# jgrss/cultionet

Hardware: AMD Instinct MI355X
Metric: train_chips_per_sec (higher is better)
Workload: dtype f32

## Files before the change

### cultionet_amd/csrc/cn_wgrad.hip

```cpp
#include <cstdlib>
#include "cn_common.h"
#include "cn_profile.h"
#include "cn_slicesum.h"

#define WG_MAX_TAPS 9
#define WG_BC 32
#define WG_NS 4
#define WG_NB 13
#define WG_KS 8
#define WG_U 4
#define WG_KB 16

struct CnWgradGeom {
  int N;
  int A, Hs, Ws; long sbs; long scs;
  int Bc, Hb, Wb; long bbs; long bcs;
  double flops;
  int s;
  int T;
  int offy[WG_MAX_TAPS], offx[WG_MAX_TAPS];
  int min_oy, min_ox;
  long sa;
  int PR, Wsp, pitch_s;
  int rows_b, pitch_b, plane_b;
  int a_tiles;
  int chunks_per_img, total_chunks, chunks_per_split;
  int b_lds_off;
  int buf_stride;
  int nbuf;
  int colsplit;
  int G, spg;
  const float* gS[4];
  const float* gB[4];
  float* gdW[4];
  long slice_stride;
  int grid_x, grid_y, grid_z;
  int mq_lo, mq_hi;
};

typedef __attribute__((address_space(3))) void* cn_lds_ptr;
typedef const __attribute__((address_space(1))) void* cn_gbl_ptr;

__device__ float cn_zero_line[64];

__device__ __forceinline__ void cn_glds4(const float* src, float* lds_wave_base) {
  __builtin_amdgcn_global_load_lds((cn_gbl_ptr)src, (cn_lds_ptr)lds_wave_base, 4, 0, 0);
}

template <int T>
__global__ __launch_bounds__(256) void cn_wgrad_kernel(const float* __restrict__ S, const float* __restrict__ Bg,
                                                      float* __restrict__ dW, const CnWgradGeom g) {
  extern __shared__ __attribute__((aligned(16))) float smem[];

  const int tid = threadIdx.x, lane = tid & 63, wid = tid >> 6;
  const int half = lane >> 5, l31 = lane & 31;
  const int at = wid % g.a_tiles, kp = wid / g.a_tiles, kparts = 4 / g.a_tiles;
  int bx, by, bz;
  if (!cn_xcd_block(g.grid_x, g.grid_y, g.grid_x * g.grid_y * g.grid_z, bx, by, bz)) return;
  const int a0 = by * g.a_tiles * 32;
  const int b0 = bx * WG_BC;
  const int npix = g.PR * g.Wsp;
  const float* zero = cn_zero_line + lane;

  int so[WG_NS];
#pragma unroll
  for (int i = 0; i < WG_NS; ++i) {
    const int e = lane + i * 64;
    if (e < npix) {
      const int r = e / g.Wsp, c = e - r * g.Wsp;
      so[i] = (r << 16) | ((c < g.Ws) ? c : 0xFFFF);
    } else {
      so[i] = -2;
    }
  }
  int bo[WG_NB];
#pragma unroll
  for (int i = 0; i < WG_NB; ++i) {
    const int e = lane + i * 64;
    if (e < g.plane_b) {
      const int r = e / g.pitch_b;
      bo[i] = (r << 16) | (e - r * g.pitch_b);
    } else {
      bo[i] = -1;
    }
  }

  int boff[T];
#pragma unroll
  for (int j = 0; j < T; ++j) {
    const int n = j * 32 + l31;
    const int bl = n / T, t = n - bl * T;
    boff[j] = bl * g.plane_b + (g.offy[t] - g.min_oy) * g.pitch_b + (g.offx[t] - g.min_ox) + half * g.s;
  }
  const int aoff = (at * 32 + l31) * g.pitch_s + half;

  f32x16 acc[T];
#pragma unroll
  for (int j = 0; j < T; ++j)
#pragma unroll
    for (int r = 0; r < 16; ++r) acc[j][r] = 0.f;

  const int HWs = g.Hs * g.Ws, HWb = g.Hb * g.Wb;
  const int arows = g.a_tiles * 32;
  int chunk = bz * g.chunks_per_split;
  int chunk_end = chunk + g.chunks_per_split;
  if (chunk_end > g.total_chunks) chunk_end = g.total_chunks;

  const int steps = npix >> 1;
  const int q_begin = (steps * kp) / kparts, q_end = (steps * (kp + 1)) / kparts;
  const int e_begin = q_begin * 2;
  const int r_begin = e_begin / g.Wsp, c_begin = e_begin - r_begin * g.Wsp;

  auto stage = [&](int ck, int buf) {
    float* s_lds = smem + buf * g.buf_stride;
    float* b_lds = s_lds + g.b_lds_off;
    const int n = ck / g.chunks_per_img;
    const int gy0 = (ck - n * g.chunks_per_img) * g.PR;
    const int pr = (g.Hs - gy0 < g.PR) ? g.Hs - gy0 : g.PR;
    const float* Sn = S + (long)n * g.sbs + (long)gy0 * g.Ws;
    for (int a = wid; a < arows; a += 4) {
      const bool aok = (a0 + a) < g.A;
      const float* Sa = Sn + (long)(a0 + a) * g.scs;
#pragma unroll
      for (int i = 0; i < WG_NS; ++i) {
        if (i * 64 < npix) {
          if (so[i] != -2) {
            const int r = so[i] >> 16, c = so[i] & 0xFFFF;
            const float* src = (aok && c != 0xFFFF && r < pr) ? Sa + r * g.Ws + c : zero;
            cn_glds4(src, s_lds + a * g.pitch_s + i * 64);
          }
        }
      }
    }
    const float* Bn = Bg + (long)n * g.bbs;
    const int iy0 = gy0 * g.s + g.min_oy;
    for (int bl = wid; bl < WG_BC; bl += 4) {
      const bool bok = (b0 + bl) < g.Bc;
      const float* Bb = Bn + (long)(b0 + bl) * g.bcs;
#pragma unroll
      for (int i = 0; i < WG_NB; ++i) {
        if (i * 64 < g.plane_b) {
          if (bo[i] >= 0) {
            const int iy = iy0 + (bo[i] >> 16), ix = g.min_ox + (bo[i] & 0xFFFF);
            const float* src = (bok && iy >= 0 && iy < g.Hb && ix >= 0 && ix < g.Wb) ? Bb + iy * g.Wb + ix : zero;
            cn_glds4(src, b_lds + bl * g.plane_b + i * 64);
          }
        }
      }
    }
  };

  int cur = 0;
  if (chunk < chunk_end && g.nbuf == 2) stage(chunk, 0);
  for (; chunk < chunk_end; ++chunk) {
    if (g.nbuf == 1) {
      __syncthreads();
      stage(chunk, 0);
    }
    __syncthreads();
    if (g.nbuf == 2 && chunk + 1 < chunk_end) stage(chunk + 1, cur ^ 1);
    const float* s_lds = smem + cur * g.buf_stride;
    const float* b_lds = s_lds + g.b_lds_off;
    int r = r_begin, c = c_begin;
    for (int q = q_begin; q < q_end; ++q) {
      const float av = s_lds[aoff + r * g.Wsp + c];
      const int bbase = (r * g.s) * g.pitch_b + c * g.s;
#pragma unroll
      for (int j = 0; j < T; ++j) {
        const float bv = b_lds[boff[j] + bbase];
        acc[j] = __builtin_amdgcn_mfma_f32_32x32x2f32(av, bv, acc[j], 0, 0, 0);
      }
      c += 2;
      if (c >= g.Wsp) { c = 0; ++r; }
    }
    if (g.nbuf == 2) cur ^= 1;
  }

#pragma unroll
  for (int j = 0; j < T; ++j) {
    const int n = j * 32 + l31;
    const int bl = n / T;
    const bool bok = (b0 + bl) < g.Bc;
#pragma unroll
    for (int r = 0; r < 16; ++r) {
      const int a = a0 + at * 32 + (r & 3) + 8 * (r >> 2) + 4 * half;
      if (bok && a < g.A) atomicAdd(dW + (long)a * g.sa + (long)b0 * T + n, acc[j][r]);
    }
  }
}

__device__ float cn_zero_line16[256];

#ifdef CNW_STAMP
__device__ unsigned long long cnw_stamps[256];
#define CNW_ST() do { if (do_stamp && stamp_i < 256) cnw_stamps[stamp_i++] = __builtin_amdgcn_s_memtime(); } while (0)
extern "C" int cn_wgrad_read_stamps(unsigned long long* out) {
  return hipMemcpyFromSymbol(out, HIP_SYMBOL(cnw_stamps), sizeof(unsigned long long) * 256) == hipSuccess ? 0 : -2;
}
#else
#define CNW_ST() do { } while (0)
#endif

__device__ __forceinline__ void cn_glds16(const float* src, float* lds_wave_base) {
  __builtin_amdgcn_global_load_lds((cn_gbl_ptr)src, (cn_lds_ptr)lds_wave_base, 16, 0, 0);
}

template <int T, int S_>
__global__ __launch_bounds__(256) void cn_wgrad_vec_kernel(const float* __restrict__ S0, const float* __restrict__ Bg0,
                                                          float* __restrict__ dW0, const CnWgradGeom g) {
  extern __shared__ __attribute__((aligned(16))) float smem[];
  const int tid = threadIdx.x, lane = tid & 63;
  const int wid = __builtin_amdgcn_readfirstlane(tid >> 6);
  const int half = lane >> 5, l31 = lane & 31;
  const int at = wid % g.a_tiles, kp = wid / g.a_tiles, kparts = 4 / g.a_tiles;
  int bx, by, bz;
  if (!cn_xcd_block(g.grid_x, g.grid_y, g.grid_x * g.grid_y * g.grid_z, bx, by, bz)) return;
  const int grp = g.G > 1 ? bz / g.spg : 0;
  const int split = bz - grp * g.spg;
  const float* __restrict__ S = g.G > 1 ? g.gS[grp] : S0;
  const float* __restrict__ Bg = g.G > 1 ? g.gB[grp] : Bg0;
  float* __restrict__ dW = (g.G > 1 && g.slice_stride == 0) ? g.gdW[grp] : dW0;
  const int a0 = by * g.a_tiles * 32;
  const int b0 = bx * WG_BC;
  const int npix = g.PR * g.Ws;
  const int n4s = npix >> 2;
  const int n4b = g.plane_b >> 2;
  const float* zero = cn_zero_line16 + 4 * lane;
  const int HWs = g.Hs * g.Ws, HWb = g.Hb * g.Wb;

  int boff[T], ox[T];
#pragma unroll
  for (int j = 0; j < T; ++j) {
    const int n = j * 32 + l31;
    const int bl = n / T, t = n - bl * T;
    boff[j] = bl * g.plane_b + (g.offy[t] - g.min_oy) * g.Wb + (g.offx[t] - g.min_ox) + half * g.s;
    ox[j] = g.offx[t] + half * g.s;
  }
  const int aoff = (at * 32 + l31) * g.pitch_s + half;

  f32x16 acc[T];
#pragma unroll
  for (int j = 0; j < T; ++j)
#pragma unroll
    for (int r = 0; r < 16; ++r) acc[j][r] = 0.f;

  const int arows = g.a_tiles * 32;
  int chunk = split * g.chunks_per_split;
  int chunk_end = chunk + g.chunks_per_split;
  if (chunk_end > g.total_chunks) chunk_end = g.total_chunks;

  const int steps = npix >> 1;
  const int q_begin = (steps * kp) / kparts, q_end = (steps * (kp + 1)) / kparts;
  const int e_begin = q_begin * 2;
  const int r_begin = e_begin / g.Ws, c_begin = e_begin - r_begin * g.Ws;

  constexpr unsigned WG_IDLE = 0xFFFFFFFFu;
  unsigned so[WG_KS], bo[WG_KB];
  {
    const int nsp = arows * n4s, nbp = WG_BC * n4b;
#pragma unroll
    for (int k = 0; k < WG_KS; ++k) {
      const int p = (wid + 4 * k) * 64 + lane;
      const int a = p / n4s, pc = p - a * n4s;
      so[k] = (p < nsp && (a0 + a) < g.A) ? (unsigned)(((long)(a0 + a) * g.scs + 4 * pc) * 4) : WG_IDLE;
    }
#pragma unroll
    for (int k = 0; k < WG_KB; ++k) {
      const int p = (wid + 4 * k) * 64 + lane;
      const int bl = p / n4b, pi = p - bl * n4b;
      bo[k] = (p < nbp && (b0 + bl) < g.Bc) ? (unsigned)(((long)(b0 + bl) * g.bcs + 4 * pi) * 4) : WG_IDLE;
    }
  }
  auto stage = [&](int ck, int buf) {
    float* s_lds = smem + buf * g.buf_stride;
    float* b_lds = s_lds + g.b_lds_off;
    const int n = ck / g.chunks_per_img;
    const int gy0 = (ck - n * g.chunks_per_img) * g.PR;
    const int nsp = arows * n4s, nbp = WG_BC * n4b;
    {
      const int fs0 = gy0 * g.Ws;
      const char* sbase = reinterpret_cast<const char*>(S + (long)n * g.sbs + fs0);
      if (fs0 + npix <= (int)g.scs) {
#pragma unroll
        for (int k = 0; k < WG_KS; ++k)
          if ((wid + 4 * k) * 64 < nsp && so[k] != WG_IDLE)
            cn_glds16(reinterpret_cast<const float*>(sbase + so[k]), s_lds + (wid + 4 * k) * 256);
      } else {
#pragma unroll
        for (int k = 0; k < WG_KS; ++k) {
          if ((wid + 4 * k) * 64 < nsp && so[k] != WG_IDLE) {
            const int p = (wid + 4 * k) * 64 + lane;
            const int pc = p % n4s;
            const bool ok = (fs0 + 4 * pc + 3) < (int)g.scs;
            const float* src = ok ? reinterpret_cast<const float*>(sbase + so[k]) : zero;
            cn_glds16(src, s_lds + (wid + 4 * k) * 256);
          }
        }
      }
    }
    {
      const int start = (gy0 * g.s + g.min_oy) * g.Wb + g.min_ox;
      const int f0 = (start >> 2) << 2;
      const char* bbase = reinterpret_cast<const char*>(Bg + (long)n * g.bbs + f0);
      if (f0 >= 0 && f0 + g.plane_b <= (int)g.bcs) {
#pragma unroll
        for (int k = 0; k < WG_KB; ++k)
          if ((wid + 4 * k) * 64 < nbp && bo[k] != WG_IDLE)
            cn_glds16(reinterpret_cast<const float*>(bbase + bo[k]), b_lds + (wid + 4 * k) * 256);
      } else {
#pragma unroll
        for (int k = 0; k < WG_KB; ++k) {
          if ((wid + 4 * k) * 64 < nbp && bo[k] != WG_IDLE) {
            const int p = (wid + 4 * k) * 64 + lane;
            const int fq = f0 + 4 * (p % n4b);
            const bool ok = fq >= 0 && (fq + 3) < (int)g.bcs;
            const float* src = ok ? reinterpret_cast<const float*>(bbase + bo[k]) : zero;
            cn_glds16(src, b_lds + (wid + 4 * k) * 256);
          }
        }
      }
    }
  };

  int cur = 0;
#ifdef CNW_STAMP
  const bool do_stamp = T == 9 && S_ == 1 && blockIdx.x == 8 && tid == 0;
  int stamp_i = 0;
#endif
  CNW_ST();
  if (chunk < chunk_end && g.nbuf == 2) stage(chunk, 0);
  for (; chunk < chunk_end; ++chunk) {
    CNW_ST();
    if (g.nbuf == 1) {
      __syncthreads();
      stage(chunk, 0);
    }
    __syncthreads();
    CNW_ST();
    if (g.nbuf == 2 && chunk + 1 < chunk_end) stage(chunk + 1, cur ^ 1);
    CNW_ST();
    const float* s_lds = smem + cur * g.buf_stride;
    const float* b_lds = s_lds + g.b_lds_off;
    const int gy0c = (chunk % g.chunks_per_img) * g.PR;
    const int start = (gy0c * g.s + g.min_oy) * g.Wb + g.min_ox;
    const int sh = start - ((start >> 2) << 2);
    {
      const int nq_row = g.Ws >> 1;
      const int q_lo = (nq_row * kp) / kparts, q_hi = (nq_row * (kp + 1)) / kparts;
      const int seg0 = min(max(g.mq_lo, q_lo), q_hi), seg1 = max(min(g.mq_hi, q_hi), seg0);
      for (int r = 0; r < g.PR; ++r) {
        const float* ap = s_lds + aoff + r * g.Ws;
        const float* bp[T];
#pragma unroll
        for (int j = 0; j < T; ++j) bp[j] = b_lds + boff[j] + sh + (r * S_) * g.Wb;
        int q = q_lo;
        for (; q < seg0; ++q) {
          const float av = ap[2 * q];
          const int cs = 2 * q * S_;
          float bv[T];
#pragma unroll
          for (int j = 0; j < T; ++j) bv[j] = bp[j][cs];
#pragma unroll
          for (int j = 0; j < T; ++j) {
            const float b_ = ((unsigned)(cs + ox[j]) < (unsigned)g.Wb) ? bv[j] : 0.f;
            acc[j] = __builtin_amdgcn_mfma_f32_32x32x2f32(av, b_, acc[j], 0, 0, 0);
          }
        }
        CNW_ST();
        if constexpr (T == 1) {
          for (; q + WG_U <= seg1; q += WG_U) {
            const float* apq = ap + 2 * q;
#pragma unroll
            for (int u = 0; u < WG_U; ++u)
              acc[0] = __builtin_amdgcn_mfma_f32_32x32x2f32(apq[2 * u], (bp[0] + 2 * q * S_)[2 * u * S_], acc[0], 0, 0, 0);
          }
        } else {
          constexpr int GS = 2;
          const int ng = (seg1 - q) / GS;
          if (ng > 0) {
            float a0[GS], a1[GS], b0[GS][T], b1[GS][T];
#define WG_LOADG(qq_, a_, b_)                                                    \
  {                                                                              \
    const float* apq_ = ap + 2 * (qq_);                                          \
    _Pragma("unroll") for (int u = 0; u < GS; ++u) a_[u] = apq_[2 * u];          \
    _Pragma("unroll") for (int j = 0; j < T; ++j) {                              \
      const float* bq_ = bp[j] + 2 * (qq_) * S_;                                 \
      _Pragma("unroll") for (int u = 0; u < GS; ++u) b_[u][j] = bq_[2 * u * S_]; \
    }                                                                            \
  }
#define WG_MFMAG(a_, b_)                                                                                   \
  {                                                                                                        \
    _Pragma("unroll") for (int u = 0; u < GS; ++u)                                                         \
        _Pragma("unroll") for (int j = 0; j < T; ++j)                                                      \
            acc[j] = __builtin_amdgcn_mfma_f32_32x32x2f32(a_[u], b_[u][j], acc[j], 0, 0, 0);               \
  }
            WG_LOADG(q, a0, b0);
            int i = 0;
            for (; i + 2 <= ng; i += 2) {
              WG_LOADG(q + GS * (i + 1), a1, b1);
              WG_MFMAG(a0, b0);
              if (i + 2 < ng) WG_LOADG(q + GS * (i + 2), a0, b0);
              WG_MFMAG(a1, b1);
            }
            if (i < ng) WG_MFMAG(a0, b0);
#undef WG_LOADG
#undef WG_MFMAG
            q += GS * ng;
          }
        }
        CNW_ST();
        for (; q < seg1; ++q) {
          const float av = ap[2 * q];
          float bv[T];
#pragma unroll
          for (int j = 0; j < T; ++j) bv[j] = bp[j][2 * q * S_];
#pragma unroll
          for (int j = 0; j < T; ++j) acc[j] = __builtin_amdgcn_mfma_f32_32x32x2f32(av, bv[j], acc[j], 0, 0, 0);
        }
        for (; q < q_hi; ++q) {
          const float av = ap[2 * q];
          const int cs = 2 * q * S_;
          float bv[T];
#pragma unroll
          for (int j = 0; j < T; ++j) bv[j] = bp[j][cs];
#pragma unroll
          for (int j = 0; j < T; ++j) {
            const float b_ = ((unsigned)(cs + ox[j]) < (unsigned)g.Wb) ? bv[j] : 0.f;
            acc[j] = __builtin_amdgcn_mfma_f32_32x32x2f32(av, b_, acc[j], 0, 0, 0);
          }
        }
      }
    }
    CNW_ST();
    if (g.nbuf == 2) cur ^= 1;
  }
  CNW_ST();

  if (kparts > 1) {
    __syncthreads();
    float* red = smem;
    if (kp > 0) {
      float* rp = red + (long)((kp - 1) * g.a_tiles + at) * (T * 16 * 64) + lane;
#pragma unroll
      for (int j = 0; j < T; ++j)
#pragma unroll
        for (int r = 0; r < 16; ++r) rp[(j * 16 + r) * 64] = acc[j][r];
    }
    __syncthreads();
    if (kp > 0) return;
    for (int k = 1; k < kparts; ++k) {
      const float* rp = red + (long)((k - 1) * g.a_tiles + at) * (T * 16 * 64) + lane;
#pragma unroll
      for (int j = 0; j < T; ++j)
#pragma unroll
        for (int r = 0; r < 16; ++r) acc[j][r] += rp[(j * 16 + r) * 64];
    }
  }
  float* dWs = dW + (long)bz * g.slice_stride;
#pragma unroll
  for (int j = 0; j < T; ++j) {
    const int n = j * 32 + l31;
    const int bl = n / T;
    const bool bok = (b0 + bl) < g.Bc;
#pragma unroll
    for (int r = 0; r < 16; ++r) {
      const int a = a0 + at * 32 + (r & 3) + 8 * (r >> 2) + 4 * half;
      if (bok && a < g.A) {
        if (g.slice_stride != 0) dWs[(long)a * g.sa + (long)b0 * T + n] = acc[j][r];
        else atomicAdd(dW + (long)a * g.sa + (long)b0 * T + n, acc[j][r]);
      }
    }
  }
}

#define WG3_WAVES 12
#define WG3_KS 3
#define WG3_KB 6
template <int S_>
__global__ __launch_bounds__(WG3_WAVES * 64) void cn_wgrad_vec3_kernel(const float* __restrict__ S0,
                                                                       const float* __restrict__ Bg0,
                                                                       float* __restrict__ dW0, const CnWgradGeom g) {
  extern __shared__ __attribute__((aligned(16))) float smem[];
  constexpr int T = 3;
  const int tid = threadIdx.x, lane = tid & 63;
  const int wid = __builtin_amdgcn_readfirstlane(tid >> 6);
  const int half = lane >> 5, l31 = lane & 31;
  const int at = wid % g.a_tiles;
  const int ky = (wid / g.a_tiles) % 3;
  const int kp = wid / (g.a_tiles * 3), kparts = WG3_WAVES / (g.a_tiles * 3);
  int bx, by, bz;
  if (!cn_xcd_block(g.grid_x, g.grid_y, g.grid_x * g.grid_y * g.grid_z, bx, by, bz)) return;
  const int grp = g.G > 1 ? bz / g.spg : 0;
  const int split = bz - grp * g.spg;
  const float* __restrict__ S = g.G > 1 ? g.gS[grp] : S0;
  const float* __restrict__ Bg = g.G > 1 ? g.gB[grp] : Bg0;
  float* __restrict__ dW = (g.G > 1 && g.slice_stride == 0) ? g.gdW[grp] : dW0;
  const int a0 = by * g.a_tiles * 32;
  const int b0 = bx * WG_BC;
  const int npix = g.PR * g.Ws;
  const int n4s = npix >> 2;
  const int n4b = g.plane_b >> 2;
  const float* zero = cn_zero_line16 + 4 * lane;

  int boff[T], ox[T];
#pragma unroll
  for (int j = 0; j < T; ++j) {
    const int n = j * 32 + l31;
    const int bl = n / 3, t = ky * 3 + (n - bl * 3);
    boff[j] = bl * g.plane_b + (g.offy[t] - g.min_oy) * g.Wb + (g.offx[t] - g.min_ox) + half * g.s;
    ox[j] = g.offx[t] + half * g.s;
  }
  const int aoff = (at * 32 + l31) * g.pitch_s + half;

  f32x16 acc[T];
#pragma unroll
  for (int j = 0; j < T; ++j)
#pragma unroll
    for (int r = 0; r < 16; ++r) acc[j][r] = 0.f;

  const int arows = g.a_tiles * 32;
  int chunk = split * g.chunks_per_split;
  int chunk_end = chunk + g.chunks_per_split;
  if (chunk_end > g.total_chunks) chunk_end = g.total_chunks;

  constexpr unsigned WG_IDLE = 0xFFFFFFFFu;
  unsigned so[WG3_KS], bo[WG3_KB];
  {
    const int nsp = arows * n4s, nbp = WG_BC * n4b;
#pragma unroll
    for (int k = 0; k < WG3_KS; ++k) {
      const int p = (wid + WG3_WAVES * k) * 64 + lane;
      const int a = p / n4s, pc = p - a * n4s;
      so[k] = (p < nsp && (a0 + a) < g.A) ? (unsigned)(((long)(a0 + a) * g.scs + 4 * pc) * 4) : WG_IDLE;
    }
#pragma unroll
    for (int k = 0; k < WG3_KB; ++k) {
      const int p = (wid + WG3_WAVES * k) * 64 + lane;
      const int bl = p / n4b, pi = p - bl * n4b;
      bo[k] = (p < nbp && (b0 + bl) < g.Bc) ? (unsigned)(((long)(b0 + bl) * g.bcs + 4 * pi) * 4) : WG_IDLE;
    }
  }
  auto stage = [&](int ck, int buf) {
    float* s_lds = smem + buf * g.buf_stride;
    float* b_lds = s_lds + g.b_lds_off;
    const int n = ck / g.chunks_per_img;
    const int gy0 = (ck - n * g.chunks_per_img) * g.PR;
    const int nsp = arows * n4s, nbp = WG_BC * n4b;
    {
      const int fs0 = gy0 * g.Ws;
      const char* sbase = reinterpret_cast<const char*>(S + (long)n * g.sbs + fs0);
      const bool inside = fs0 + npix <= (int)g.scs;
#pragma unroll
      for (int k = 0; k < WG3_KS; ++k) {
        if ((wid + WG3_WAVES * k) * 64 < nsp && so[k] != WG_IDLE) {
          const float* src = reinterpret_cast<const float*>(sbase + so[k]);
          if (!inside) {
            const int p = (wid + WG3_WAVES * k) * 64 + lane;
            if (!((fs0 + 4 * (p % n4s) + 3) < (int)g.scs)) src = zero;
          }
          cn_glds16(src, s_lds + (wid + WG3_WAVES * k) * 256);
        }
      }
    }
    {
      const int start = (gy0 * g.s + g.min_oy) * g.Wb + g.min_ox;
      const int f0 = (start >> 2) << 2;
      const char* bbase = reinterpret_cast<const char*>(Bg + (long)n * g.bbs + f0);
      const bool inside = f0 >= 0 && f0 + g.plane_b <= (int)g.bcs;
#pragma unroll
      for (int k = 0; k < WG3_KB; ++k) {
        if ((wid + WG3_WAVES * k) * 64 < nbp && bo[k] != WG_IDLE) {
          const float* src = reinterpret_cast<const float*>(bbase + bo[k]);
          if (!inside) {
            const int p = (wid + WG3_WAVES * k) * 64 + lane;
            const int fq = f0 + 4 * (p % n4b);
            if (!(fq >= 0 && (fq + 3) < (int)g.bcs)) src = zero;
          }
          cn_glds16(src, b_lds + (wid + WG3_WAVES * k) * 256);
        }
      }
    }
  };

  int cur = 0;
  if (chunk < chunk_end && g.nbuf == 2) stage(chunk, 0);
  for (; chunk < chunk_end; ++chunk) {
    if (g.nbuf == 1) {
      __syncthreads();
      stage(chunk, 0);
    }
    __syncthreads();
    if (g.nbuf == 2 && chunk + 1 < chunk_end) stage(chunk + 1, cur ^ 1);
    const float* s_lds = smem + cur * g.buf_stride;
    const float* b_lds = s_lds + g.b_lds_off;
    const int gy0c = (chunk % g.chunks_per_img) * g.PR;
    const int start = (gy0c * g.s + g.min_oy) * g.Wb + g.min_ox;
    const int sh = start - ((start >> 2) << 2);
    const int nq_row = g.Ws >> 1;
    const int q_lo = (nq_row * kp) / kparts, q_hi = (nq_row * (kp + 1)) / kparts;
    const int seg0 = min(max(g.mq_lo, q_lo), q_hi), seg1 = max(min(g.mq_hi, q_hi), seg0);
    for (int r = 0; r < g.PR; ++r) {
      const float* ap = s_lds + aoff + r * g.Ws;
      const float* bp[T];
#pragma unroll
      for (int j = 0; j < T; ++j) bp[j] = b_lds + boff[j] + sh + (r * S_) * g.Wb;
      int q = q_lo;
      for (; q < seg0; ++q) {
        const float av = ap[2 * q];
        const int cs = 2 * q * S_;
        float bv[T];
#pragma unroll
        for (int j = 0; j < T; ++j) bv[j] = bp[j][cs];
#pragma unroll
        for (int j = 0; j < T; ++j) {
          const float b_ = ((unsigned)(cs + ox[j]) < (unsigned)g.Wb) ? bv[j] : 0.f;
          acc[j] = __builtin_amdgcn_mfma_f32_32x32x2f32(av, b_, acc[j], 0, 0, 0);
        }
      }
      {
        constexpr int GS = 3;
        const int ng = (seg1 - q) / GS;
        if (ng > 0) {
          float a0[GS], a1[GS], b0[GS][T], b1[GS][T];
#define WG3_LOADG(qq_, a_, b_)                                                   \
  {                                                                              \
    const float* apq_ = ap + 2 * (qq_);                                          \
    _Pragma("unroll") for (int u = 0; u < GS; ++u) a_[u] = apq_[2 * u];          \
    _Pragma("unroll") for (int j = 0; j < T; ++j) {                              \
      const float* bq_ = bp[j] + 2 * (qq_) * S_;                                 \
      _Pragma("unroll") for (int u = 0; u < GS; ++u) b_[u][j] = bq_[2 * u * S_]; \
    }                                                                            \
  }
#define WG3_MFMAG(a_, b_)                                                                                  \
  {                                                                                                        \
    _Pragma("unroll") for (int u = 0; u < GS; ++u)                                                         \
        _Pragma("unroll") for (int j = 0; j < T; ++j)                                                      \
            acc[j] = __builtin_amdgcn_mfma_f32_32x32x2f32(a_[u], b_[u][j], acc[j], 0, 0, 0);               \
  }
          WG3_LOADG(q, a0, b0);
          int i = 0;
          for (; i + 2 <= ng; i += 2) {
            WG3_LOADG(q + GS * (i + 1), a1, b1);
            WG3_MFMAG(a0, b0);
            if (i + 2 < ng) WG3_LOADG(q + GS * (i + 2), a0, b0);
            WG3_MFMAG(a1, b1);
          }
          if (i < ng) WG3_MFMAG(a0, b0);
#undef WG3_LOADG
#undef WG3_MFMAG
          q += GS * ng;
        }
      }
      for (; q < seg1; ++q) {
        const float av = ap[2 * q];
        float bv[T];
#pragma unroll
        for (int j = 0; j < T; ++j) bv[j] = bp[j][2 * q * S_];
#pragma unroll
        for (int j = 0; j < T; ++j) acc[j] = __builtin_amdgcn_mfma_f32_32x32x2f32(av, bv[j], acc[j], 0, 0, 0);
      }
      for (; q < q_hi; ++q) {
        const float av = ap[2 * q];
        const int cs = 2 * q * S_;
        float bv[T];
#pragma unroll
        for (int j = 0; j < T; ++j) bv[j] = bp[j][cs];
#pragma unroll
        for (int j = 0; j < T; ++j) {
          const float b_ = ((unsigned)(cs + ox[j]) < (unsigned)g.Wb) ? bv[j] : 0.f;
          acc[j] = __builtin_amdgcn_mfma_f32_32x32x2f32(av, b_, acc[j], 0, 0, 0);
        }
      }
    }
    if (g.nbuf == 2) cur ^= 1;
  }

  if (kparts > 1) {
    __syncthreads();
    float* red = smem;
    const int slot = ky * g.a_tiles + at;
    if (kp > 0) {
      float* rp = red + (long)((kp - 1) * g.a_tiles * 3 + slot) * (T * 16 * 64) + lane;
#pragma unroll
      for (int j = 0; j < T; ++j)
#pragma unroll
        for (int r = 0; r < 16; ++r) rp[(j * 16 + r) * 64] = acc[j][r];
    }
    __syncthreads();
    if (kp > 0) return;
    for (int k = 1; k < kparts; ++k) {
      const float* rp = red + (long)((k - 1) * g.a_tiles * 3 + slot) * (T * 16 * 64) + lane;
#pragma unroll
      for (int j = 0; j < T; ++j)
#pragma unroll
        for (int r = 0; r < 16; ++r) acc[j][r] += rp[(j * 16 + r) * 64];
    }
  }
  float* dWs = dW + (long)bz * g.slice_stride;
#pragma unroll
  for (int j = 0; j < T; ++j) {
    const int n = j * 32 + l31;
    const int bl = n / 3, t = ky * 3 + (n - bl * 3);
    const bool bok = (b0 + bl) < g.Bc;
#pragma unroll
    for (int r = 0; r < 16; ++r) {
      const int a = a0 + at * 32 + (r & 3) + 8 * (r >> 2) + 4 * half;
      if (bok && a < g.A) {
        float* d = (g.slice_stride != 0 ? dWs : dW) + (long)a * g.sa + (long)(b0 + bl) * 9 + t;
        if (g.slice_stride != 0) *d = acc[j][r];
        else atomicAdd(d, acc[j][r]);
      }
    }
  }
}

struct CnWgradReduceArgs {
  const float* part; long slice_stride; int nslices; long n;
  float* dW[4];
};
__global__ __launch_bounds__(256) void cn_wgrad_reduce_kernel(const CnWgradReduceArgs a) {
  const long i = blockIdx.x * 256L + threadIdx.x;
  if (i >= a.n) return;
  const float* part = a.part + (long)blockIdx.z * a.nslices * a.slice_stride;
  float* dW = a.dW[blockIdx.z];
  float s0 = 0.f, s1 = 0.f;
  int k = blockIdx.y;
  for (; k + (int)gridDim.y < a.nslices; k += 2 * gridDim.y) {
    s0 += part[(long)k * a.slice_stride + i];
    s1 += part[(long)(k + gridDim.y) * a.slice_stride + i];
  }
  if (k < a.nslices) s0 += part[(long)k * a.slice_stride + i];
  if (gridDim.y == 1) dW[i] += s0 + s1;
  else atomicAdd(dW + i, s0 + s1);
}

template <int T>
static int cn_wgrad_launch_vec(const float* S, const float* Bg, float* dW, CnWgradGeom g, float* ws, long ws_floats,
                               hipStream_t stream) {
  if (g.scs % 4 || g.bcs % 4 || g.sbs % 4 || g.bbs % 4 || (g.Ws & 1)) return CN_ERR_ARG;
  g.Wsp = g.Ws;
  g.PR = 128 / g.Ws;
  if (g.PR < 1) g.PR = 1;
  if (g.PR > g.Hs) g.PR = g.Hs;
  while (g.PR > 1 && (g.PR * g.Ws) % 4 != 0) --g.PR;
  if ((g.PR * g.Ws) % 4 != 0 && g.Ws % 2 == 0 && 2 * g.Ws <= 256) g.PR = 2;
  if ((g.PR * g.Ws) % 4 != 0 || g.PR * g.Ws > 256) return CN_ERR_ARG;
  int max_oy = g.min_oy, max_ox = g.min_ox;
  for (int t = 0; t < g.T; ++t) {
    if (g.offy[t] > max_oy) max_oy = g.offy[t];
    if (g.offx[t] > max_ox) max_ox = g.offx[t];
  }
  g.rows_b = (g.PR - 1) * g.s + (max_oy - g.min_oy) + 1;
  g.pitch_b = g.Wb;
  g.plane_b = ((g.rows_b - 1) * g.Wb + (g.Ws - 1) * g.s + (max_ox - g.min_ox) + 4 + 3) / 4 * 4;
  if (WG_BC * g.plane_b > WG_KB * 4 * 256) return CN_ERR_ARG;
  g.pitch_s = g.PR * g.Ws;
  g.a_tiles = g.A > 32 ? 2 : 1;
  size_t lds;
  for (;;) {
    g.b_lds_off = (g.a_tiles * 32 * g.pitch_s + 255) / 256 * 256;
    g.buf_stride = g.b_lds_off + (WG_BC * g.plane_b + 255) / 256 * 256;
    lds = (size_t)g.buf_stride * sizeof(float);
    if ((lds <= 160 * 1024 && g.a_tiles * 32 * g.pitch_s <= WG_KS * 4 * 256) || g.a_tiles == 1) break;
    g.a_tiles >>= 1;
  }
  if (lds > 160 * 1024 || g.a_tiles * 32 * g.pitch_s > WG_KS * 4 * 256) return CN_ERR_ARG;
  g.nbuf = (2 * lds <= 160 * 1024) ? 2 : 1;
  lds *= g.nbuf;
  {
    const size_t red = (size_t)(4 / g.a_tiles - 1) * g.a_tiles * T * 16 * 64 * sizeof(float);
    if (red > lds) lds = red;
  }
  g.chunks_per_img = (g.Hs + g.PR - 1) / g.PR;
  g.total_chunks = g.N * g.chunks_per_img;
  const int gx = (g.Bc + WG_BC - 1) / WG_BC, gy = (g.A + g.a_tiles * 32 - 1) / (g.a_tiles * 32);
  if (g.G < 1) {
    g.G = 1;
    g.gS[0] = S; g.gB[0] = Bg; g.gdW[0] = dW;
  }
  for (int i = 0; i < g.G; ++i)
    if ((reinterpret_cast<uintptr_t>(g.gS[i]) & 15) || (reinterpret_cast<uintptr_t>(g.gB[i]) & 15)) return CN_ERR_ARG;
  const int slots = (lds * 2 <= 160 * 1024) ? 512 : 256;
  int splits = slots / (gx * gy * g.G);
  if (splits > g.total_chunks) splits = g.total_chunks;
  if (splits < 1) splits = 1;
  g.chunks_per_split = (g.total_chunks + splits - 1) / splits;
  splits = (g.total_chunks + g.chunks_per_split - 1) / g.chunks_per_split;
  static bool attr_set = false;
  if (!attr_set) {
    (void)hipFuncSetAttribute((const void*)cn_wgrad_vec_kernel<T, 1>, hipFuncAttributeMaxDynamicSharedMemorySize,
                              160 * 1024);
    (void)hipFuncSetAttribute((const void*)cn_wgrad_vec_kernel<T, 2>, hipFuncAttributeMaxDynamicSharedMemorySize,
                              160 * 1024);
    attr_set = true;
  }
  if (g.s != 1 && g.s != 2) return CN_ERR_ARG;
  {
    const int nq_row = g.Ws / 2;
    int lo = (-g.min_ox + 2 * g.s - 1) / (2 * g.s);
    if (lo < 0) lo = 0;
    int hi_num = g.Wb - max_ox - g.s;
    int hi = hi_num <= 0 ? 0 : (hi_num + 2 * g.s - 1) / (2 * g.s);
    if (lo > nq_row) lo = nq_row;
    if (hi > nq_row) hi = nq_row;
    if (hi < lo) hi = lo;
    g.mq_lo = lo;
    g.mq_hi = hi;
  }
  cn_prof_name("cn_wgrad_vec_kernel<%d, %d>", T, g.s == 1 ? 1 : 2);
  cn_prof_desc("wgrad_vec<%d> G%d N%d A%d %dx%d Bc%d %dx%d s%d grid%dx%dx%d nbuf%d", T, g.G, g.N, g.A, g.Hs, g.Ws, g.Bc,
               g.Hb, g.Wb, g.s, gx, gy, splits, g.nbuf);
  g.spg = splits;
  g.grid_x = gx; g.grid_y = gy; g.grid_z = splits * g.G;
  const dim3 grid(cn_xcd_grid((long)gx * gy * splits * g.G));
  const int kparts = 4 / g.a_tiles;
  const long dw_floats = (long)g.A * g.sa;
  const long nslices = splits;
  float* out = g.gdW[0];
  g.slice_stride = 0;
  if (nslices >= 16 && ws != nullptr && nslices * g.G * dw_floats <= ws_floats) {
    g.slice_stride = dw_floats;
    out = ws;
  }
  if (T == 9) cn_prof_name("cn_wgrad_vec3_kernel<%d>", g.s == 1 ? 1 : 2);
  cn_prof_bytes(4.0 * g.G * ((double)g.N * g.A * g.Hs * g.Ws + (double)g.N * g.Bc * g.Hb * g.Wb + (double)dw_floats));
  cn_prof_before(stream);
  if (T == 9) {
    static bool attr3 = false;
    if (!attr3) {
      (void)hipFuncSetAttribute((const void*)cn_wgrad_vec3_kernel<1>, hipFuncAttributeMaxDynamicSharedMemorySize, 160 * 1024);
      (void)hipFuncSetAttribute((const void*)cn_wgrad_vec3_kernel<2>, hipFuncAttributeMaxDynamicSharedMemorySize, 160 * 1024);
      attr3 = true;
    }
    if (g.s == 1)
      CN_LAUNCH((cn_wgrad_vec3_kernel<1>), grid, dim3(WG3_WAVES * 64), lds, stream, g.gS[0], g.gB[0], out, g);
    else
      CN_LAUNCH((cn_wgrad_vec3_kernel<2>), grid, dim3(WG3_WAVES * 64), lds, stream, g.gS[0], g.gB[0], out, g);
  } else if (g.s == 1)
    CN_LAUNCH((cn_wgrad_vec_kernel<T, 1>), grid, dim3(256), lds, stream, g.gS[0], g.gB[0], out, g);
  else
    CN_LAUNCH((cn_wgrad_vec_kernel<T, 2>), grid, dim3(256), lds, stream, g.gS[0], g.gB[0], out, g);
  cn_prof_after(stream, T == 9 ? 2 : 3, g.flops * g.G);
  if (g.slice_stride != 0) {
    CnSliceSum js[4] = {};
    for (int i = 0; i < g.G; ++i) {
      js[i].part = ws + (long)i * nslices * g.slice_stride; js[i].dw = g.gdW[i]; js[i].slice_stride = g.slice_stride;
      js[i].n = dw_floats; js[i].nslices = (int)nslices; js[i].kind = 0;
    }
    if (cn_ss_push(js, g.G)) return cn_check_launch();
    CnWgradReduceArgs ra = {ws, g.slice_stride, (int)nslices, dw_floats, {g.gdW[0], g.gdW[1], g.gdW[2], g.gdW[3]}};
    CN_LAUNCH(cn_wgrad_reduce_kernel,
                       dim3((unsigned)((dw_floats + 255) / 256), nslices > 128 ? 16 : 1, g.G), dim3(256), 0, stream,
                       ra);
  }
  return cn_check_launch();
}

template <int T>
static int cn_wgrad_launch_t(const float* S, const float* Bg, float* dW, CnWgradGeom g, hipStream_t stream) {
  g.Wsp = (g.Ws + 1) & ~1;
  if (g.Wsp > 64 * WG_NS) return CN_ERR_LDS;
  g.PR = 128 / g.Wsp;
  if (g.PR < 1) g.PR = 1;
  if (g.PR > g.Hs) g.PR = g.Hs;
  int max_oy = g.min_oy, max_ox = g.min_ox;
  for (int t = 0; t < g.T; ++t) {
    if (g.offy[t] > max_oy) max_oy = g.offy[t];
    if (g.offx[t] > max_ox) max_ox = g.offx[t];
  }
  for (;;) {
    g.rows_b = (g.PR - 1) * g.s + (max_oy - g.min_oy) + 1;
    g.pitch_b = (g.Wsp - 1) * g.s + (max_ox - g.min_ox) + 1;
    g.plane_b = g.rows_b * g.pitch_b;
    if (g.plane_b <= 64 * WG_NB || g.PR == 1) break;
    --g.PR;
  }
  if (g.plane_b > 64 * WG_NB) return CN_ERR_LDS;
  g.pitch_s = (g.PR * g.Wsp) | 1;
  g.a_tiles = g.A > 64 ? 4 : (g.A > 32 ? 2 : 1);
  if (g.a_tiles == 4) g.a_tiles = 2;
  size_t lds;
  for (;;) {
    g.b_lds_off = (g.a_tiles * 32 * g.pitch_s + 3) / 4 * 4;
    g.buf_stride = (g.b_lds_off + WG_BC * g.plane_b + 3) / 4 * 4;
    lds = (size_t)g.buf_stride * sizeof(float);
    if (lds <= 160 * 1024 || g.a_tiles == 1) break;
    g.a_tiles >>= 1;
  }
  if (lds > 160 * 1024) return CN_ERR_LDS;
  g.nbuf = (2 * lds <= 160 * 1024) ? 2 : 1;
  lds *= g.nbuf;
  g.chunks_per_img = (g.Hs + g.PR - 1) / g.PR;
  g.total_chunks = g.N * g.chunks_per_img;
  const int gx = (g.Bc + WG_BC - 1) / WG_BC, gy = (g.A + g.a_tiles * 32 - 1) / (g.a_tiles * 32);
  int splits = (768 + gx * gy - 1) / (gx * gy);
  if (splits > g.total_chunks) splits = g.total_chunks;
  if (splits < 1) splits = 1;
  g.chunks_per_split = (g.total_chunks + splits - 1) / splits;
  splits = (g.total_chunks + g.chunks_per_split - 1) / g.chunks_per_split;
  static bool attr_set = false;
  if (!attr_set) {
    (void)hipFuncSetAttribute((const void*)cn_wgrad_kernel<T>, hipFuncAttributeMaxDynamicSharedMemorySize,
                              160 * 1024);
    attr_set = true;
  }
  cn_prof_name("cn_wgrad_kernel<%d>", T);
  cn_prof_desc("wgrad_dw<%d> N%d A%d %dx%d Bc%d %dx%d s%d grid%dx%dx%d", T, g.N, g.A, g.Hs, g.Ws, g.Bc, g.Hb, g.Wb, g.s,
               gx, gy, splits);
  g.grid_x = gx; g.grid_y = gy; g.grid_z = splits;
  cn_prof_before(stream);
  CN_LAUNCH((cn_wgrad_kernel<T>), dim3(cn_xcd_grid((long)gx * gy * splits)), dim3(256), lds, stream, S, Bg,
                     dW, g);
  cn_prof_after(stream, T == 9 ? 2 : 3, g.flops);
  return cn_check_launch();
}

struct CnPadSet {
  const float* src; long sbs; long scs;
  float* dst; int C, H, W, Wp, cs;
};
#define CN_PAD_MAX_SETS 8
struct CnPadArgs {
  CnPadSet set[CN_PAD_MAX_SETS];
  int cbegin[CN_PAD_MAX_SETS + 1];
  int nsets;
};

__global__ __launch_bounds__(256) void cn_pad_planes_kernel(const CnPadArgs a) {
  int si = 0;
#pragma unroll 1
  for (int i = 1; i < a.nsets; ++i)
    if ((int)blockIdx.y >= a.cbegin[i]) si = i;
  const CnPadSet& p = a.set[si];
  const int c = blockIdx.y - a.cbegin[si], b = blockIdx.z;
  const float* sp = p.src + b * p.sbs + (long)c * p.scs;
  float* dp = p.dst + ((long)b * p.C + c) * p.cs;
  for (int i = blockIdx.x * 256 + threadIdx.x; i < p.cs; i += gridDim.x * 256) {
    const int r = i / p.Wp, col = i - r * p.Wp;
    dp[i] = (r < p.H && col < p.W) ? sp[r * p.W + col] : 0.f;
  }
}

static int cn_pad_planes(CnPadArgs& a, int B, hipStream_t stream) {
  if (a.nsets == 0) return CN_OK;
  int cs = 0, ctot = 0;
  for (int i = 0; i < a.nsets; ++i) {
    a.cbegin[i] = ctot;
    ctot += a.set[i].C;
    if (a.set[i].cs > cs) cs = a.set[i].cs;
  }
  a.cbegin[a.nsets] = ctot;
  int bx = (cs + 1023) / 1024;
  if (bx < 1) bx = 1;
  CN_LAUNCH(cn_pad_planes_kernel, dim3(bx, ctot, B), dim3(256), 0, stream, a);
  return cn_check_launch();
}

static int cn_wgrad_generic_g(int G, const float* const* Ss, long sbs, int A, int Hs, int Ws, const float* const* Bgs,
                              long bbs, int Bc, int Hb, int Wb, int s, int KH, int KW, int dil, int pad,
                              float* const* dWs, int N, float* ws, long ws_floats, hipStream_t stream) {
  if (G < 1 || G > 4) return CN_ERR_ARG;
  CnWgradGeom g = {};
  g.N = N; g.A = A; g.Hs = Hs; g.Ws = Ws; g.sbs = sbs; g.Bc = Bc; g.Hb = Hb; g.Wb = Wb; g.bbs = bbs; g.s = s;
  g.scs = (long)Hs * Ws; g.bcs = (long)Hb * Wb;
  g.T = KH * KW;
  if (N <= 0 || A <= 0 || Bc <= 0 || Hs <= 0 || Ws <= 0) return CN_OK;
  g.flops = 2.0 * N * Hs * Ws * (double)A * Bc * g.T;
  for (int ky = 0; ky < KH; ++ky)
    for (int kx = 0; kx < KW; ++kx) {
      g.offy[ky * KW + kx] = ky * dil - pad;
      g.offx[ky * KW + kx] = kx * dil - pad;
    }
  g.min_oy = -pad; g.min_ox = -pad;
  g.sa = (long)Bc * g.T;
  if (g.T != 1 && g.T != 9) return CN_ERR_ARG;
  g.G = G;
  for (int i = 0; i < G; ++i) { g.gS[i] = Ss[i]; g.gB[i] = Bgs[i]; g.gdW[i] = dWs[i]; }
  const bool ws_ok = ws != nullptr && (reinterpret_cast<uintptr_t>(ws) & 15) == 0;
  int rc = g.T == 1 ? cn_wgrad_launch_vec<1>(Ss[0], Bgs[0], dWs[0], g, ws_ok ? ws : nullptr, ws_floats, stream)
                    : cn_wgrad_launch_vec<9>(Ss[0], Bgs[0], dWs[0], g, ws_ok ? ws : nullptr, ws_floats, stream);
  if (rc != CN_ERR_ARG) return rc;
  if (ws_ok) {
    const int Wsp = (Ws + 1) & ~1;
    const long scs = ((long)Hs * Wsp + 3) / 4 * 4, bcs = ((long)Hb * Wb + 3) / 4 * 4;
    const long need_s = (long)N * A * scs, need_b = (long)N * Bc * bcs;
    CnWgradGeom gp = g;
    CnPadArgs pa = {};
    float* w = ws;
    long need = 0;
    bool any_s = false, any_b = false;
    for (int i = 0; i < G; ++i) {
      const bool s_ok = (g.scs % 4 == 0) && (sbs % 4 == 0) && !(Ws & 1) && !(reinterpret_cast<uintptr_t>(Ss[i]) & 15);
      const bool b_ok = (g.bcs % 4 == 0) && (bbs % 4 == 0) && !(reinterpret_cast<uintptr_t>(Bgs[i]) & 15);
      any_s |= !s_ok;
      any_b |= !b_ok;
    }
    for (int i = 0; i < G && any_s; ++i) {
      pa.set[pa.nsets++] = {Ss[i], sbs, (long)Hs * Ws, w, A, Hs, Ws, Wsp, (int)scs};
      gp.gS[i] = w; w += need_s; need += need_s;
    }
    for (int i = 0; i < G && any_b; ++i) {
      int same = -1;
      for (int j = 0; j < i; ++j)
        if (Bgs[j] == Bgs[i]) same = j;
      if (same >= 0) { gp.gB[i] = gp.gB[same]; continue; }
      pa.set[pa.nsets++] = {Bgs[i], bbs, (long)Hb * Wb, w, Bc, Hb, Wb, Wb, (int)bcs};
      gp.gB[i] = w; w += need_b; need += need_b;
    }
    if (any_s) { gp.Ws = Wsp; gp.scs = scs; gp.sbs = (long)A * scs; }
    if (any_b) { gp.bcs = bcs; gp.bbs = (long)Bc * bcs; }
    if (need <= ws_floats) {
      const int r = cn_pad_planes(pa, N, stream);
      if (r != CN_OK) return r;
      float* wrest = ws + (need + 3) / 4 * 4;
      const long nrest = ws_floats - (need + 3) / 4 * 4;
      rc = g.T == 1 ? cn_wgrad_launch_vec<1>(gp.gS[0], gp.gB[0], dWs[0], gp, wrest, nrest, stream)
                    : cn_wgrad_launch_vec<9>(gp.gS[0], gp.gB[0], dWs[0], gp, wrest, nrest, stream);
      if (rc != CN_ERR_ARG) return rc;
    }
  }
  for (int i = 0; i < G; ++i) {
    CnWgradGeom g1 = g;
    g1.G = 0;
    rc = g.T == 1 ? cn_wgrad_launch_t<1>(Ss[i], Bgs[i], dWs[i], g1, stream)
                  : cn_wgrad_launch_t<9>(Ss[i], Bgs[i], dWs[i], g1, stream);
    if (rc != CN_OK) return rc;
  }
  return CN_OK;
}

static int cn_wgrad_generic(const float* S, long sbs, int A, int Hs, int Ws, const float* Bg, long bbs, int Bc,
                            int Hb, int Wb, int s, int KH, int KW, int dil, int pad, float* dW, int N, float* ws,
                            long ws_floats, hipStream_t stream) {
  return cn_wgrad_generic_g(1, &S, sbs, A, Hs, Ws, &Bg, bbs, Bc, Hb, Wb, s, KH, KW, dil, pad, &dW, N, ws, ws_floats,
                            stream);
}

extern "C" int cn_conv2d_bwd_weight_grouped_f32(int G, const float* const* xs, long xbs, const float* const* dys,
                                                long dybs, float* const* dws, int B, int Cin, int Hin, int Win,
                                                int Cout, int KH, int KW, int stride, int pad, int dil, float* ws,
                                                long ws_floats, void* stream) {
  if (stride < 1) return CN_ERR_ARG;
  const int Hout = (Hin + 2 * pad - dil * (KH - 1) - 1) / stride + 1;
  const int Wout = (Win + 2 * pad - dil * (KW - 1) - 1) / stride + 1;
  return cn_wgrad_generic_g(G, dys, dybs, Cout, Hout, Wout, xs, xbs, Cin, Hin, Win, stride, KH, KW, dil, pad, dws, B,
                            ws, ws_floats, (hipStream_t)stream);
}

extern "C" int cn_conv2d_bwd_weight_f32(const float* x, long xbs, const float* dy, long dybs, float* dw, int B,
                                        int Cin, int Hin, int Win, int Cout, int KH, int KW, int stride, int pad,
                                        int dil, float* ws, long ws_floats, void* stream) {
  if (stride < 1) return CN_ERR_ARG;
  const int Hout = (Hin + 2 * pad - dil * (KH - 1) - 1) / stride + 1;
  const int Wout = (Win + 2 * pad - dil * (KW - 1) - 1) / stride + 1;
  return cn_wgrad_generic(dy, dybs, Cout, Hout, Wout, x, xbs, Cin, Hin, Win, stride, KH, KW, dil, pad, dw, B, ws,
                          ws_floats, (hipStream_t)stream);
}

extern "C" int cn_conv_transpose2d_bwd_weight_f32(const float* x, long xbs, const float* dy, long dybs, float* dw,
                                                  int B, int Cin, int Hin, int Win, int Cout, int KH, int KW,
                                                  int stride, int pad, int out_pad, float* ws, long ws_floats,
                                                  void* stream) {
  if (out_pad < 0 || (out_pad > 0 && out_pad >= stride)) return CN_ERR_ARG;
  const int Hout = (Hin - 1) * stride - 2 * pad + KH + out_pad;
  const int Wout = (Win - 1) * stride - 2 * pad + KW + out_pad;
  return cn_wgrad_generic(x, xbs, Cin, Hin, Win, dy, dybs, Cout, Hout, Wout, stride, KH, KW, 1, pad, dw, B, ws,
                          ws_floats, (hipStream_t)stream);
}
```

Baseline: 391.4.

## Add MFMA GEMM path for stride-1 1x1 conv weight gradients

Adds a dedicated weight-gradient kernel for 1x1, stride-1, unpadded convolutions. It treats each image's flattened spatial extent as the K dimension and runs a tiled MFMA GEMM with double-buffered LDS staging through global_load_lds. The reduction is split across chunks, with optional per-split partial slices reduced by a separate kernel and k-parts summed through LDS. This replaces the more general tap-based vec kernel for this case, at the cost of a new code path with its own tiling and split heuristics.

```diff
diff --git a/cultionet_amd/csrc/cn_wgrad.hip b/cultionet_amd/csrc/cn_wgrad.hip
--- a/cultionet_amd/csrc/cn_wgrad.hip
+++ b/cultionet_amd/csrc/cn_wgrad.hip
@@ -36,6 +36,7 @@
   long slice_stride;
   int grid_x, grid_y, grid_z;
   int mq_lo, mq_hi;
+  int flat_n;
 };
 
 typedef __attribute__((address_space(3))) void* cn_lds_ptr;
@@ -734,6 +735,226 @@
   else atomicAdd(dW + i, s0 + s1);
 }
 
+#define WGG_KC 68
+#define WGG_P4 (WGG_KC / 4)
+template <int WM, int WN, int KP>
+__global__ __launch_bounds__(64 * WM * WN * KP) __attribute__((amdgpu_waves_per_eu(2, 2))) void cn_wgrad_gemm_kernel(const float* __restrict__ S,
+                                                                          const float* __restrict__ Bg,
+                                                                          float* __restrict__ dW, const CnWgradGeom g) {
+  extern __shared__ __attribute__((aligned(16))) float smem[];
+  constexpr int NW = WM * WN * KP, TM = 64 * WM, TN = 64 * WN, ROWS = TM + TN;
+  constexpr int NI = ROWS * WGG_P4 / 64;
+  constexpr int NIS = TM * WGG_P4 / 64;
+  constexpr int KI = (NI + NW - 1) / NW;
+  constexpr int BUF = ROWS * WGG_KC;
+  constexpr int NS = 8 / KP;
+  static_assert(WGG_KC == 68 && 8 % KP == 0, "a chunk is 8 eight-float steps and one four-float tail");
+  const int tid = threadIdx.x, lane = tid & 63;
+  const int wid = __builtin_amdgcn_readfirstlane(tid >> 6);
+  const int half = lane >> 5, l31 = lane & 31;
+  const int kp = wid / (WM * WN), wt = wid % (WM * WN), wm = wt % WM, wn = wt / WM;
+  int bx, by, bz;
+  if (!cn_xcd_block(g.grid_x, g.grid_y, g.grid_x * g.grid_y * g.grid_z, bx, by, bz)) return;
+  const int a0 = by * TM, b0 = bx * TN;
+  const float* zero = cn_zero_line16 + 4 * lane;
+
+  constexpr unsigned WG_IDLE = 0xFFFFFFFFu;
+  unsigned so[KI];
+#pragma unroll
+  for (int k = 0; k < KI; ++k) {
+    const int i = wid + NW * k;
+    const int p = i * 64 + lane;
+    const int row = p / WGG_P4, pc = p - row * WGG_P4;
+    if (i < NIS) so[k] = (a0 + row) < g.A ? (unsigned)(((long)(a0 + row) * g.scs + 4 * pc) * 4) : WG_IDLE;
+    else so[k] = (b0 + row - TM) < g.Bc ? (unsigned)(((long)(b0 + row - TM) * g.bcs + 4 * pc) * 4) : WG_IDLE;
+  }
+  auto stage = [&](int ck, int buf) {
+    float* lds = smem + buf * BUF;
+    const int n = ck / g.chunks_per_img;
+    const int f0 = (ck - n * g.chunks_per_img) * WGG_KC;
+    const char* sbase = reinterpret_cast<const char*>(S + (long)n * g.sbs + f0);
+    const char* bbase = reinterpret_cast<const char*>(Bg + (long)n * g.bbs + f0);
+    const bool inside = f0 + WGG_KC <= g.flat_n;
+#pragma unroll
+    for (int k = 0; k < KI; ++k) {
+      const int i = wid + NW * k;
+      if (i < NI) {
+        const float* src = so[k] != WG_IDLE ? reinterpret_cast<const float*>((i < NIS ? sbase : bbase) + so[k]) : zero;
+        if (!inside) {
+          const int pc = (i * 64 + lane) % WGG_P4;
+          if (f0 + 4 * pc + 4 > g.flat_n) src = zero;
+        }
+        cn_glds16(src, lds + i * 256);
+      }
+    }
+  };
+
+  f32x16 acc[2][2];
+#pragma unroll
+  for (int i = 0; i < 2; ++i)
+#pragma unroll
+    for (int j = 0; j < 2; ++j)
+#pragma unroll
+      for (int r = 0; r < 16; ++r) acc[i][j][r] = 0.f;
+
+  int chunk = bz * g.chunks_per_split;
+  int chunk_end = chunk + g.chunks_per_split;
+  if (chunk_end > g.total_chunks) chunk_end = g.total_chunks;
+  const int aoff = (wm * 64 + l31) * WGG_KC + kp * NS * 8 + 4 * half;
+  const int boff = (TM + wn * 64 + l31) * WGG_KC + kp * NS * 8 + 4 * half;
+  const int atail = (wm * 64 + l31) * WGG_KC + 64 + 2 * half;
+  const int btail = (TM + wn * 64 + l31) * WGG_KC + 64 + 2 * half;
+
+  int cur = 0;
+  if (chunk < chunk_end) stage(chunk, 0);
+  for (; chunk < chunk_end; ++chunk) {
+    __syncthreads();
+    if (chunk + 1 < chunk_end) stage(chunk + 1, cur ^ 1);
+    const float* lds = smem + cur * BUF;
+    const float* ap = lds + aoff;
+    const float* bp = lds + boff;
+    f32x4 va[2][2], vb[2][2];
+#define WGG_LOAD(s_, u_)                                                                     \
+  {                                                                                          \
+    va[s_][0] = *reinterpret_cast<const f32x4*>(ap + 8 * (u_));                              \
+    va[s_][1] = *reinterpret_cast<const f32x4*>(ap + 32 * WGG_KC + 8 * (u_));                \
+    vb[s_][0] = *reinterpret_cast<const f32x4*>(bp + 8 * (u_));                              \
+    vb[s_][1] = *reinterpret_cast<const f32x4*>(bp + 32 * WGG_KC + 8 * (u_));                \
+  }
+    WGG_LOAD(0, 0);
+#pragma unroll
+    for (int u = 0; u < NS; ++u) {
+      if (u + 1 < NS) WGG_LOAD((u + 1) & 1, u + 1);
+#pragma unroll
+      for (int e = 0; e < 4; ++e)
+#pragma unroll
+        for (int i = 0; i < 2; ++i)
+#pragma unroll
+          for (int j = 0; j < 2; ++j)
+            acc[i][j] = __builtin_amdgcn_mfma_f32_32x32x2f32(va[u & 1][i][e], vb[u & 1][j][e], acc[i][j], 0, 0, 0);
+    }
+#undef WGG_LOAD
+    if (kp == KP - 1) {
+      f32x2 ta[2], tb[2];
+      ta[0] = *reinterpret_cast<const f32x2*>(lds + atail);
+      ta[1] = *reinterpret_cast<const f32x2*>(lds + atail + 32 * WGG_KC);
+      tb[0] = *reinterpret_cast<const f32x2*>(lds + btail);
+      tb[1] = *reinterpret_cast<const f32x2*>(lds + btail + 32 * WGG_KC);
+#pragma unroll
+      for (int e = 0; e < 2; ++e)
+#pragma unroll
+        for (int i = 0; i < 2; ++i)
+#pragma unroll
+          for (int j = 0; j < 2; ++j)
+            acc[i][j] = __builtin_amdgcn_mfma_f32_32x32x2f32(ta[i][e], tb[j][e], acc[i][j], 0, 0, 0);
+    }
+    cur ^= 1;
+  }
+
+  if (KP > 1) {
+    __syncthreads();
+    float* red = smem;
+    if (kp > 0) {
+      float* rp = red + (long)((kp - 1) * WM * WN + wt) * (4 * 16 * 64) + lane;
+#pragma unroll
+      for (int t = 0; t < 4; ++t)
+#pragma unroll
+        for (int r = 0; r < 16; ++r) rp[(t * 16 + r) * 64] = acc[t >> 1][t & 1][r];
+    }
+    __syncthreads();
+    if (kp > 0) return;
+#pragma unroll 1
+    for (int k = 1; k < KP; ++k) {
+      const float* rp = red + (long)((k - 1) * WM * WN + wt) * (4 * 16 * 64) + lane;
+#pragma unroll
+      for (int t = 0; t < 4; ++t)
+#pragma unroll
+        for (int r = 0; r < 16; ++r) acc[t >> 1][t & 1][r] += rp[(t * 16 + r) * 64];
+    }
+  }
+  float* out = dW + (long)bz * g.slice_stride;
+#pragma unroll
+  for (int i = 0; i < 2; ++i)
+#pragma unroll
+    for (int j = 0; j < 2; ++j) {
+      const int b = b0 + wn * 64 + j * 32 + l31;
+#pragma unroll
+      for (int r = 0; r < 16; ++r) {
+        const int a = a0 + wm * 64 + i * 32 + (r & 3) + 8 * (r >> 2) + 4 * half;
+        if (a < g.A && b < g.Bc) {
+          if (g.slice_stride != 0) out[(long)a * g.sa + b] = acc[i][j][r];
+          else atomicAdd(dW + (long)a * g.sa + b, acc[i][j][r]);
+        }
+      }
+    }
+}
+
+template <int WM, int WN, int KP>
+static void cn_wgrad_gemm_go(const float* S, const float* Bg, float* out, const CnWgradGeom& g, hipStream_t stream) {
+  constexpr size_t lds = (size_t)2 * 64 * (WM + WN) * WGG_KC * sizeof(float);
+  static_assert(lds >= (size_t)(KP - 1) * WM * WN * 4 * 16 * 64 * sizeof(float), "the k-part sums reuse the buffers");
+  static bool attr_set = false;
+  if (!attr_set) {
+    (void)hipFuncSetAttribute((const void*)cn_wgrad_gemm_kernel<WM, WN, KP>, hipFuncAttributeMaxDynamicSharedMemorySize,
+                              (int)lds);
+    attr_set = true;
+  }
+  CN_LAUNCH((cn_wgrad_gemm_kernel<WM, WN, KP>), dim3(cn_xcd_grid((long)g.grid_x * g.grid_y * g.grid_z)),
+            dim3(64 * WM * WN * KP), lds, stream, S, Bg, out, g);
+}
+
+static int cn_wgrad_launch_gemm(const float* S, const float* Bg, float* dW, CnWgradGeom g, float* ws, long ws_floats,
+                                hipStream_t stream) {
+  if (g.T != 1 || g.s != 1 || g.G != 1 || g.min_oy != 0 || g.min_ox != 0 || g.Hs != g.Hb || g.Ws != g.Wb)
+    return CN_ERR_ARG;
+  if (g.scs % 4 || g.bcs % 4 || g.sbs % 4 || g.bbs % 4) return CN_ERR_ARG;
+  if ((reinterpret_cast<uintptr_t>(S) & 15) || (reinterpret_cast<uintptr_t>(Bg) & 15)) return CN_ERR_ARG;
+  const long hw = (long)g.Hs * g.Ws;
+  g.flat_n = (int)((hw + 3) / 4 * 4);
+  if (g.scs < g.flat_n || g.bcs < g.flat_n) return CN_ERR_ARG;
+  if ((long)g.A * g.scs >= (1L << 30) || (long)g.Bc * g.bcs >= (1L << 30)) return CN_ERR_ARG;
+  g.chunks_per_img = (int)((hw + WGG_KC - 1) / WGG_KC);
+  g.total_chunks = g.N * g.chunks_per_img;
+  int tile = 128, slots = 256;
+  for (;;) {
+    g.grid_x = (g.Bc + tile - 1) / tile;
+    g.grid_y = (g.A + tile - 1) / tile;
+    int splits = slots / (g.grid_x * g.grid_y);
+    if (splits > g.total_chunks) splits = g.total_chunks;
+    if (splits < 1) splits = 1;
+    g.chunks_per_split = (g.total_chunks + splits - 1) / splits;
+    g.grid_z = (g.total_chunks + g.chunks_per_split - 1) / g.chunks_per_split;
+    if (tile == 64 || g.chunks_per_split >= 8) break;
+    tile = 64; slots = 512;
+  }
+  const int splits = g.grid_z;
+  g.spg = splits;
+  const long dw_floats = (long)g.A * g.sa;
+  float* out = dW;
+  g.slice_stride = 0;
+  if (splits >= 16 && ws != nullptr && splits * dw_floats <= ws_floats) {
+    g.slice_stride = dw_floats;
+    out = ws;
+  }
+  cn_prof_name("cn_wgrad_gemm_kernel<%d>", tile);
+  cn_prof_desc("wgrad_gemm N%d A%d %dx%d Bc%d tile%d grid%dx%dx%d", g.N, g.A, g.Hs, g.Ws, g.Bc, tile, g.grid_x, g.grid_y,
+               splits);
+  cn_prof_bytes(4.0 * ((double)g.N * (g.A + g.Bc) * hw + (double)dw_floats));
+  cn_prof_before(stream);
+  if (tile == 128) cn_wgrad_gemm_go<2, 2, 2>(S, Bg, out, g, stream);
+  else cn_wgrad_gemm_go<1, 1, 4>(S, Bg, out, g, stream);
+  cn_prof_after(stream, 3, g.flops);
+  if (g.slice_stride != 0) {
+    CnSliceSum js = {};
+    js.part = ws; js.dw = dW; js.slice_stride = g.slice_stride; js.n = dw_floats; js.nslices = splits; js.kind = 0;
+    if (cn_ss_push(&js, 1)) return cn_check_launch();
+    CnWgradReduceArgs ra = {ws, g.slice_stride, splits, dw_floats, {dW, nullptr, nullptr, nullptr}};
+    CN_LAUNCH(cn_wgrad_reduce_kernel, dim3((unsigned)((dw_floats + 255) / 256), splits > 128 ? 16 : 1, 1), dim3(256), 0,
+              stream, ra);
+  }
+  return cn_check_launch();
+}
+
 template <int T>
 static int cn_wgrad_launch_vec(const float* S, const float* Bg, float* dW, CnWgradGeom g, float* ws, long ws_floats,
                                hipStream_t stream) {
@@ -977,11 +1198,13 @@
   g.G = G;
   for (int i = 0; i < G; ++i) { g.gS[i] = Ss[i]; g.gB[i] = Bgs[i]; g.gdW[i] = dWs[i]; }
   const bool ws_ok = ws != nullptr && (reinterpret_cast<uintptr_t>(ws) & 15) == 0;
-  int rc = g.T == 1 ? cn_wgrad_launch_vec<1>(Ss[0], Bgs[0], dWs[0], g, ws_ok ? ws : nullptr, ws_floats, stream)
+  const bool gemm = G == 1 && g.T == 1 && s == 1 && pad == 0 && Hs == Hb && Ws == Wb;
+  int rc = gemm     ? cn_wgrad_launch_gemm(Ss[0], Bgs[0], dWs[0], g, ws_ok ? ws : nullptr, ws_floats, stream)
+         : g.T == 1 ? cn_wgrad_launch_vec<1>(Ss[0], Bgs[0], dWs[0], g, ws_ok ? ws : nullptr, ws_floats, stream)
                     : cn_wgrad_launch_vec<9>(Ss[0], Bgs[0], dWs[0], g, ws_ok ? ws : nullptr, ws_floats, stream);
   if (rc != CN_ERR_ARG) return rc;
   if (ws_ok) {
-    const int Wsp = (Ws + 1) & ~1;
+    const int Wsp = gemm ? Ws : (Ws + 1) & ~1;
     const long scs = ((long)Hs * Wsp + 3) / 4 * 4, bcs = ((long)Hb * Wb + 3) / 4 * 4;
     const long need_s = (long)N * A * scs, need_b = (long)N * Bc * bcs;
     CnWgradGeom gp = g;
@@ -990,7 +1213,8 @@
     long need = 0;
     bool any_s = false, any_b = false;
     for (int i = 0; i < G; ++i) {
-      const bool s_ok = (g.scs % 4 == 0) && (sbs % 4 == 0) && !(Ws & 1) && !(reinterpret_cast<uintptr_t>(Ss[i]) & 15);
+      const bool s_ok = (g.scs % 4 == 0) && (sbs % 4 == 0) && (gemm || !(Ws & 1)) &&
+                        !(reinterpret_cast<uintptr_t>(Ss[i]) & 15);
       const bool b_ok = (g.bcs % 4 == 0) && (bbs % 4 == 0) && !(reinterpret_cast<uintptr_t>(Bgs[i]) & 15);
       any_s |= !s_ok;
       any_b |= !b_ok;
@@ -1014,7 +1238,8 @@
       if (r != CN_OK) return r;
       float* wrest = ws + (need + 3) / 4 * 4;
       const long nrest = ws_floats - (need + 3) / 4 * 4;
-      rc = g.T == 1 ? cn_wgrad_launch_vec<1>(gp.gS[0], gp.gB[0], dWs[0], gp, wrest, nrest, stream)
+      rc = gemm     ? cn_wgrad_launch_gemm(gp.gS[0], gp.gB[0], dWs[0], gp, wrest, nrest, stream)
+         : g.T == 1 ? cn_wgrad_launch_vec<1>(gp.gS[0], gp.gB[0], dWs[0], gp, wrest, nrest, stream)
                     : cn_wgrad_launch_vec<9>(gp.gS[0], gp.gB[0], dWs[0], gp, wrest, nrest, stream);
       if (rc != CN_ERR_ARG) return rc;
     }
```

After: 391.1 (median of 3 runs). No clear change (-0.1%).
